# Spandan7724/Audio-Watermarking-Deep-Learning-Watermarks-for-Authenticating-Speech

Hardware: AMD Instinct MI355X
Metric: 1-s@16kHz clips/sec (gen+det+loss fwd-bwd) (higher is better)
Workload: dtype f32; 1 GPU; main16 train step: Generator+Detector+6 losses fwd-bwd + Adam, B=256 clips/GPU x 1 GPU, 1-s @ 16 kHz, message_bits=16 (BASELINE configs[2]); batch_per_gpu=256, global_batch=256, clip_len=16000, optimizer=fused flat Adam (wm_adam_step), parallelism=single

## Files before the change

audio-watermarking-deep-learning-watermarks-for-authenticating-speech_amd/csrc/small_convs.hip:

```cpp
#include "wm_common.hpp"
using namespace wm;

namespace {

__global__ __launch_bounds__(256) void stem_fwd_kernel(const float* __restrict__ s, const float* __restrict__ w,
                                                       const float* __restrict__ bias, float* __restrict__ y, int T) {
    __shared__ float ss[1024 + 8];
    __shared__ float ws[64 * 8];
    const int tilesPerClip = (T + 1023) / 1024;
    const int b = blockIdx.x / tilesPerClip, t0 = (blockIdx.x % tilesPerClip) * 1024;
    const float* sb = s + (size_t)b * T;
    for (int i = threadIdx.x; i < 1024 + 6; i += 256) {
        const int t = t0 - 3 + i;
        ss[i] = (t >= 0 && t < T) ? sb[t] : 0.f;
    }
    for (int i = threadIdx.x; i < 512; i += 256) {
        const int co = i >> 3, j = i & 7;
        ws[i] = (j < 7) ? w[co * 7 + j] : bias[co];
    }
    __syncthreads();
    const int t = t0 + 4 * threadIdx.x;
    if (t >= T) return;
    float v[10];
#pragma unroll
// ... 372 lines not shown
    for (int i = tid; i < OB * 64; i += 256) ws[i] = (i < NO * 64) ? w[i] : 0.f;
    for (int i = tid; i < 256 * GS; i += 256) gsm[i] = 0.f;
    const int tilesPerClip = (T + 255) / 256, ntiles = B * tilesPerClip;
    f32x16 accw[NT][2];
#pragma unroll
    for (int mt = 0; mt < NT; ++mt)
#pragma unroll
        for (int r = 0; r < 16; ++r) { accw[mt][0][r] = 0.f; accw[mt][1][r] = 0.f; }
    float accb = 0.f;
    constexpr int NG4 = (256 * NOMAX + 3) / 4, NGV = (NG4 + 255) / 256;
    float4 sx[16], sgv[NGV];
    auto load_piece = [&](int tile, int p) {
        const int b = tile / tilesPerClip, t0 = (tile % tilesPerClip) * 256;
        if (p < 16) {
            const int i = tid + p * 256, c = i >> 6, q = i & 63;
            sx[p] = *reinterpret_cast<const float4*>(x + ((size_t)b * 64 + c) * T + min(t0 + 4 * q, T - 4));
        } else {
            const float4* gb4 = reinterpret_cast<const float4*>(g + ((size_t)b * T + t0) * NO);
            const int lim4 = ((T - t0 < 256 ? T - t0 : 256) * NO) / 4;
            sgv[p - 16] = gb4[min(tid + (p - 16) * 256, lim4 - 1)];
        }
    };
    auto load_tile = [&](int tile) {
#pragma unroll
        for (int p = 0; p < 16 + NGV; ++p) load_piece(tile, p);
    };
    auto write_tile = [&](int tile) {
        const int t0 = (tile % tilesPerClip) * 256;
        const int nt = min(256, T - t0);
        const int row = tile / tilesPerClip;
        long long msg = 0;
        if constexpr (DL) msg = (row < BL) ? message[row] : 0;
        const float yl = row < BL ? 1.f : 0.f;
#pragma unroll
        for (int k = 0; k < 16; ++k) {
            const int i = tid + k * 256, c = i >> 6, q = i & 63;
            float4 v = sx[k];
            if (4 * q >= nt) v = make_float4(0.f, 0.f, 0.f, 0.f);
            float* d = xs + c * XS + 4 * q;
            d[0] = v.x; d[1] = v.y; d[2] = v.z; d[3] = v.w;
        }
#pragma unroll
        for (int k = 0; k < NGV; ++k) {
            const int f = tid + k * 256;
            if (f < NG4) {
                const float e[4] = {sgv[k].x, sgv[k].y, sgv[k].z, sgv[k].w};
#pragma unroll
                for (int j = 0; j < 4; ++j) {
                    const int i = 4 * f + j;
                    if (i < 256 * NO) {
                        const int r = NOC > 0 ? i / NO : div_small(i, magic), o = i - r * NO;
                        float val = e[j];
                        if constexpr (DL) {
                            if (o == 0) val = bce_logits_grad(val, yl, kl);
                            else val = (row < BL) ? bce_logits_grad(val, (float)((msg >> (o - 1)) & 1), kb) : 0.f;
                        }
                        gsm[r * GS + o] = (i < nt * NO) ? val : 0.f;
                    }
                }
            }
        }
    };
    int tile = blockIdx.x;
    if (tile < ntiles) load_tile(tile);
    __syncthreads();
    if (tile < ntiles) write_tile(tile);
    __syncthreads();
    while (tile < ntiles) {
        const int next = tile + gridDim.x, nextc = min(next, ntiles - 1);
        const int b = tile / tilesPerClip, t0 = (tile % tilesPerClip) * 256;
        const int nt = min(256, T - t0);
        {
            f32x16 acc[2][2];
#pragma unroll
            for (int mt = 0; mt < 2; ++mt)
#pragma unroll
                for (int n2 = 0; n2 < 2; ++n2)
#pragma unroll
                    for (int r = 0; r < 16; ++r) acc[mt][n2][r] = 0.f;
#pragma unroll
            for (int s = 0; s < (NOMAX + 1) / 2; ++s) {
                if (s < KS) {
                    const float a0 = ws[(2 * s + half) * 64 + l31], a1 = ws[(2 * s + half) * 64 + 32 + l31];
                    const float b0 = gsm[(wave * 64 + l31) * GS + 2 * s + half], b1 = gsm[(wave * 64 + 32 + l31) * GS + 2 * s + half];
                    acc[0][0] = mfma32(a0, b0, acc[0][0]); acc[0][1] = mfma32(a0, b1, acc[0][1]);
                    acc[1][0] = mfma32(a1, b0, acc[1][0]); acc[1][1] = mfma32(a1, b1, acc[1][1]);
                }
            }
            float* dxb = dx + (size_t)b * 64 * T + t0;
#pragma unroll
            for (int mt = 0; mt < 2; ++mt)
#pragma unroll
                for (int n2 = 0; n2 < 2; ++n2)
#pragma unroll
                    for (int r = 0; r < 16; ++r) {
                        const int c = mt * 32 + mfma_row(r, half), tt = wave * 64 + n2 * 32 + l31;
                        if (tt < nt) dxb[(size_t)c * T + tt] = acc[mt][n2][r];
                    }
        }
        {
            const float* ap = gsm + (wave * 64 + half) * GS + l31;
            const float* bp = xs + l31 * XS + wave * 64 + half;
#pragma unroll
            for (int s = 0; s < 32; ++s) {
                if (s < 16 + NGV) load_piece(nextc, s);
#pragma unroll
                for (int mt = 0; mt < NT; ++mt) {
                    const float a = ap[2 * s * GS + mt * 32];
                    accw[mt][0] = mfma32(a, bp[2 * s], accw[mt][0]);
                    accw[mt][1] = mfma32(a, bp[32 * XS + 2 * s], accw[mt][1]);
                }
            }
        }
        if ((tid & (OB - 1)) < NO) {
            const float* gp = gsm + (tid / OB) * OB * GS + (tid & (OB - 1));
#pragma unroll 8
            for (int tt = 0; tt < OB; ++tt) accb += gp[tt * GS];
        }
        __syncthreads();
        if (next < ntiles) write_tile(next);
        __syncthreads();
        tile = next;
    }
    __syncthreads();
    float* red = xs;
    for (int wv = 0; wv < 4; ++wv) {
        if (wave == wv) {
#pragma unroll
            for (int mt = 0; mt < NT; ++mt)
#pragma unroll
                for (int n2 = 0; n2 < 2; ++n2)
#pragma unroll
                    for (int r = 0; r < 16; ++r) {
                        const int o = mt * 32 + mfma_row(r, half), c = n2 * 32 + l31;
                        red[o * 64 + c] = (wv == 0) ? accw[mt][n2][r] : red[o * 64 + c] + accw[mt][n2][r];
                    }
        }
        __syncthreads();
    }
    float* out = partial + (size_t)blockIdx.x * (NO * 64 + NO);
    for (int i = tid; i < NO * 64; i += 256) out[i] = red[i];
    __syncthreads();
    red[tid] = ((tid & (OB - 1)) < NO) ? accb : 0.f;
    __syncthreads();
    if (tid < NO) {
        if constexpr (NT == 1)
            out[NO * 64 + tid] = ((red[tid] + red[32 + tid]) + (red[64 + tid] + red[96 + tid])) +
                                 ((red[128 + tid] + red[160 + tid]) + (red[192 + tid] + red[224 + tid]));
        else
            out[NO * 64 + tid] = (red[tid] + red[64 + tid]) + (red[128 + tid] + red[192 + tid]);
    }
}

}

extern "C" {

int wm_stem_fwd(const float* s, const float* w, const float* bias, float* y, int B, int T, hipStream_t stream) {
    if (T & 3) return (int)hipErrorInvalidValue;
    hipLaunchKernelGGL(stem_fwd_kernel, dim3(B * ((T + 1023) / 1024)), dim3(256), 0, stream, s, w, bias, y, T);
    WM_CHECK_LAUNCH();
    return 0;
}

#ifndef WM_STEM_WGS_PER_CU
#define WM_STEM_WGS_PER_CU 2
#endif
int wm_stem_bwd(const float* g, const float* s, const float* w, float* ds, float* partial, float* dw, float* db, int B,
                int T, int nds, int accumulate, hipStream_t stream) {
    if (T & 3) return (int)hipErrorInvalidValue;
    constexpr size_t lds = (size_t)(64 * 264 + 296 + 4 * 256) * sizeof(float);
    static wm::DevOnce attr_done;
    if (int rc = wm::lds_opt_in(reinterpret_cast<const void*>(stem_bwd_kernel), lds, attr_done)) return rc;
    const int ntiles = B * ((T + 255) / 256);
    const int grid = ntiles < WM_STEM_WGS_PER_CU * kNumCU ? ntiles : WM_STEM_WGS_PER_CU * kNumCU;
    hipLaunchKernelGGL(stem_bwd_kernel, dim3(grid), dim3(256), lds, stream, g, s, w, ds, partial, B, T, nds);
    WM_CHECK_LAUNCH();
    hipLaunchKernelGGL(stem_reduce_kernel, dim3(8), dim3(1024), 0, stream, (const float*)partial, grid, dw, db, accumulate);
    WM_CHECK_LAUNCH();
    return 0;
}

int wm_head1_fwd(const float* x, const float* w, const float* bias, float* y, int B, int T, hipStream_t stream) {
    if (T & 3) return (int)hipErrorInvalidValue;
    const int total4 = B * (T / 4);
    hipLaunchKernelGGL(head1_fwd_kernel, dim3((total4 + 255) / 256), dim3(256), 0, stream, x, w, bias, y, T / 4, total4);
    WM_CHECK_LAUNCH();
    return 0;
}

int wm_head1_tail_fwd(const float* x, const float* y2, const float* scale, const float* shift, const float* w, const float* bias,
                      float* out, void* mask, float* y, int B, int T, hipStream_t stream) {
    if ((T & 3) || B <= 0 || !y2 || !out) return (int)hipErrorInvalidValue;
    const int T4 = T / 4, grid = B * ((T4 + 255) / 256);
    if (mask) hipLaunchKernelGGL(head1_tail_fwd_kernel<true>, dim3(grid), dim3(256), 0, stream, x, y2, scale, shift, out, (unsigned*)mask, w, bias, y, T4);
    else hipLaunchKernelGGL(head1_tail_fwd_kernel<false>, dim3(grid), dim3(256), 0, stream, x, y2, scale, shift, out, (unsigned*)nullptr, w, bias, y, T4);
    WM_CHECK_LAUNCH();
    return 0;
}

int wm_head1_bwd(const float* g, const float* x, const float* w, float* dx, float* partial, float* dw, float* db, int B,
                 int T, int accumulate, hipStream_t stream) {
    if (T & 3) return (int)hipErrorInvalidValue;
    const int total4 = B * (T / 4);
    int grid = (total4 + 255) / 256;
    if (grid > 1024) grid = 1024;
    if (dx) hipLaunchKernelGGL(head1_bwd_kernel<true>, dim3(grid), dim3(256), 0, stream, g, x, w, dx, partial, T / 4, total4);
    else hipLaunchKernelGGL(head1_bwd_kernel<false>, dim3(grid), dim3(256), 0, stream, g, x, w, dx, partial, T / 4, total4);
    WM_CHECK_LAUNCH();
    hipLaunchKernelGGL(reduce_partials_kernel, dim3(1), dim3(256), 0, stream, (const float*)partial, grid, 65, 64, dw, accumulate);
    WM_CHECK_LAUNCH();
    hipLaunchKernelGGL(reduce_partials_kernel, dim3(1), dim3(256), 0, stream, (const float*)partial + 64, grid, 65, 1, db, accumulate);
    WM_CHECK_LAUNCH();
    return 0;
}

}

namespace {
struct HeadNFwd {
    const float *x, *y2, *scale, *shift, *w, *bias;
    float *out, *y, *partial;
    unsigned* mask;
    const long long* message;
    int BL, R, T, NO;
};
template <int NOC, bool TAIL, bool LOSS>
int launch_headN_fwd(const HeadNFwd& a, hipStream_t stream) {
    const size_t lds = (size_t)256 * (NOC > 0 ? NOC : (a.NO | 1)) * sizeof(float);
    if constexpr (NOC == 0) {
        static wm::DevOnce done;
        if (int rc = wm::lds_opt_in(reinterpret_cast<const void*>(headN_fwd_kernel<NOC, TAIL, LOSS>), 256 * 65 * sizeof(float), done)) return rc;
    }
    const unsigned magic = (unsigned)((0x100000000ull + a.NO - 1) / a.NO);
    hipLaunchKernelGGL((headN_fwd_kernel<NOC, TAIL, LOSS>), dim3(a.R * ((a.T + 255) / 256)), dim3(256), lds, stream, a.x, a.y2, a.scale,
                       a.shift, a.out, a.mask, a.w, a.bias, a.y, a.message, a.BL, a.partial, a.T, a.NO, magic);
    WM_CHECK_LAUNCH();
    return 0;
}
template <bool TAIL, bool LOSS>
int launch_headN_fwd_width(const HeadNFwd& a, hipStream_t stream) {
    if (a.NO == 17) return launch_headN_fwd<17, TAIL, LOSS>(a, stream);
    if (a.NO == 1) return launch_headN_fwd<1, TAIL, LOSS>(a, stream);
    return launch_headN_fwd<0, TAIL, LOSS>(a, stream);
}
}

extern "C" {

int wm_headN_fwd(const float* x, const float* w, const float* bias, float* y, int B, int T, int NO, hipStream_t stream) {
    if (NO < 1 || NO > 64 || B <= 0 || T <= 0) return (int)hipErrorInvalidValue;
    const HeadNFwd a{x, nullptr, nullptr, nullptr, w, bias, nullptr, y, nullptr, nullptr, nullptr, 0, B, T, NO};
    return launch_headN_fwd_width<false, false>(a, stream);
}

int wm_headN_tail_fwd(const float* x, const float* y2, const float* scale, const float* shift, const float* w, const float* bias,
                      const long long* message, int B, float* partial, float* loc_out, float* bce_out, float* out, void* mask,
                      float* logits, int R, int T, int NO, hipStream_t stream) {
    if (NO < 1 || NO > 64 || R <= 0 || T <= 0) return (int)hipErrorInvalidValue;
    if (y2 && (!scale || !shift || !out)) return (int)hipErrorInvalidValue;
    if (message && (B < 0 || B > R || !partial || !loc_out || (NO > 1 && !bce_out))) return (int)hipErrorInvalidValue;
    const HeadNFwd a{x, y2, scale, shift, w, bias, out, logits, partial, y2 ? (unsigned*)mask : nullptr, message, B, R, T, NO};
    const int rc = y2 ? (message ? launch_headN_fwd_width<true, true>(a, stream) : launch_headN_fwd_width<true, false>(a, stream))
                      : (message ? launch_headN_fwd_width<false, true>(a, stream) : launch_headN_fwd_width<false, false>(a, stream));
    if (rc || !message) return rc;
    const int grid = R * ((T + 255) / 256);
    WM_TRY((hipError_t)wm::launch_sum_scale2(partial, grid, 1.0 / ((double)R * T), loc_out, stream));
    if (NO > 1) WM_TRY((hipError_t)wm::launch_sum_scale2(partial + grid, grid, 1.0 / ((double)B * T * (NO - 1)), bce_out, stream));
    return 0;
}

}

namespace {
struct HeadNBwd {
    const float *g, *x, *w;
    float *dx, *partial;
    const long long* message;
    const float *g_loc, *g_bce;
    int BL, R, T, NO;
};
template <int NOC, int NT, bool DL>
int launch_headN_bwd(const HeadNBwd& a, int grid, hipStream_t stream) {
    constexpr size_t lds = (size_t)(64 * 257 + 256 * (32 * NT + 1) + 32 * NT * 64) * sizeof(float);
    static wm::DevOnce done;
    if (int rc = wm::lds_opt_in(reinterpret_cast<const void*>(headN_bwd_kernel<NOC, NT, DL>), lds, done)) return rc;
    const unsigned magic = a.NO > 1 ? (unsigned)((0x100000000ull + a.NO - 1) / a.NO) : 0u;
    hipLaunchKernelGGL((headN_bwd_kernel<NOC, NT, DL>), dim3(grid), dim3(256), lds, stream, a.g, a.x, a.w, a.dx, a.partial, a.R, a.T, a.NO,
                       magic, a.message, a.g_loc, a.g_bce, a.BL);
    WM_CHECK_LAUNCH();
    return 0;
}
template <bool DL>
int headN_bwd(const HeadNBwd& a, float* dw, float* db, int accumulate, hipStream_t stream) {
    const int NO = a.NO;
    if (NO < 1 || NO > 64) return (int)hipErrorInvalidValue;
    const int ntiles = a.R * ((a.T + 255) / 256);
    const int grid = ntiles < kNumCU ? ntiles : kNumCU;
    int rc;
    if (NO == 17) rc = launch_headN_bwd<17, 1, DL>(a, grid, stream);
    else if (NO == 1) rc = launch_headN_bwd<1, 1, DL>(a, grid, stream);
    else if (NO <= 32) rc = launch_headN_bwd<0, 1, DL>(a, grid, stream);
    else rc = launch_headN_bwd<0, 2, DL>(a, grid, stream);
    if (rc) return rc;
    const int n = NO * 64 + NO;
    hipLaunchKernelGGL(reduce_partials_kernel, dim3((NO * 64 + 63) / 64), dim3(256), 0, stream, (const float*)a.partial, grid, n, NO * 64, dw, accumulate);
    WM_CHECK_LAUNCH();
    hipLaunchKernelGGL(reduce_partials_kernel, dim3(1), dim3(256), 0, stream, (const float*)a.partial + NO * 64, grid, n, NO, db, accumulate);
    WM_CHECK_LAUNCH();
    return 0;
}
}

extern "C" {

int wm_headN_bwd(const float* g, const float* x, const float* w, float* dx, float* partial, float* dw, float* db, int B,
                 int T, int NO, int accumulate, hipStream_t stream) {
    const HeadNBwd a{g, x, w, dx, partial, nullptr, nullptr, nullptr, 0, B, T, NO};
    return headN_bwd<false>(a, dw, db, accumulate, stream);
}

int wm_headN_bwd_bce(const float* logits, const long long* message, const float* g_loc, const float* g_bce, const float* x,
                     const float* w, float* dx, float* partial, float* dw, float* db, int B, int R, int T, int NO, int accumulate,
                     hipStream_t stream) {
    if (!message || !g_loc || !g_bce || B < 0 || B > R) return (int)hipErrorInvalidValue;
    const HeadNBwd a{logits, x, w, dx, partial, message, g_loc, g_bce, B, R, T, NO};
    return headN_bwd<true>(a, dw, db, accumulate, stream);
}

}
```

audio-watermarking-deep-learning-watermarks-for-authenticating-speech_amd/ops.py:

```python
from __future__ import annotations

import contextlib
import os

import torch

from ._host import _chk, _chk_int, _chk_positive, _f32, _p, _seed64, _stream
from ._lib import lib

NCU = 256
BN_EPS = 1e-5
BN_MOMENTUM = 0.1


def _frames(x: torch.Tensor, name: str, ch: int) -> torch.Tensor:
    x = _chk(x, name, 3)
    if x.shape[1] != ch:
        raise ValueError(f"{name}: expected {ch} channels, got shape {tuple(x.shape)}")
    if x.shape[2] % 4 != 0:
        raise ValueError(f"{name}: clip length must be a multiple of 4 samples, got {x.shape[2]}")
    return x


_GRAD = {"on": True}
# ... 124 lines not shown
def switches(**values):
    prev = {name: _LIVE[SWITCHES[name][0]][SWITCHES[name][1]] for name in values}
    try:
        for name, value in values.items():
            set_switch(name, value)
        yield
    finally:
        for name, value in prev.items():
            set_switch(name, value)


def set_conv_bf_schedule(schedule: int):
    set_switch("schedule", schedule)


def set_conv_bf16x6(on: bool):
    set_switch("bf16x6", on)


def set_fused_backward(on: bool):
    set_switch("fused_bwd", on)


def set_mask_on_load(on: bool):
    set_switch("mask_on_load", on)


def set_bwd_f16x3(on: bool):
    set_switch("bwd_f16x3", on)


def set_fwd_f16x3(on: bool):
    set_switch("fwd_f16x3", on)


def set_eval_f16x3(on: bool):
    set_switch("eval_f16x3", on)


def pack_w64_h(w: torch.Tensor, mode: int) -> torch.Tensor:
    wph = torch.empty(2 * 3 * 4096 + 4, dtype=torch.int16, device=w.device)
    lib.wm_pack_w64_h(_p(w), _p(wph), mode, _stream())
    return wph


def set_pair_fold(on: bool):
    set_switch("pair_fold", on)


def set_resblock_one_launch(on: bool):
    set_switch("one_launch_eval", on)


def conv_bf16x6() -> bool:
    return _CONV["bf16x6"]


def pack_w64_bf(w: torch.Tensor, mode: int) -> torch.Tensor:
    wpb = torch.empty(3 * 3 * 4096, dtype=torch.int16, device=w.device)
    lib.wm_pack_w64_bf(_p(w), _p(wpb), mode, _stream())
    return wpb


def set_conv7_f16x3(on: bool):
    set_switch("conv7_f16x3", on)


def pack_w64_h7(w: torch.Tensor, mode: int) -> torch.Tensor:
    wph = torch.empty(2 * 7 * 4096 + 4, dtype=torch.int16, device=w.device)
    lib.wm_pack_w64_h7(_p(w), _p(wph), mode, _stream())
    return wph


def set_lstm_fwd_wave_specialised(on: bool):
    set_switch("lstm_fwd_ws", on)


def set_lstm_bwd_wave_specialised(on: bool):
    set_switch("lstm_bwd_ws", on)


_HEADS = {"tail_in_head": os.environ.get("WM_TAIL_IN_HEAD", "1") == "1"}


def set_tail_in_head(on: bool):
    _HEADS["tail_in_head"] = bool(on)


def read_tail_in_consumer(environ) -> bool:
    return environ.get("WM_TAIL_IN_CONSUMER", "1") == "1"


_TAILC = {"on": read_tail_in_consumer(os.environ)}


def set_tail_in_consumer(on: bool):
    _TAILC["on"] = bool(on)


def read_lstm_dx_in_bwd(environ) -> bool:
    return environ.get("WM_LSTM_DX_IN_BWD", "1") == "1"


_LSTM_DX = {"in_bwd": read_lstm_dx_in_bwd(os.environ)}


def set_lstm_dx_in_bwd(on: bool):
    _LSTM_DX["in_bwd"] = bool(on)


def read_head1_rank1(environ) -> bool:
    return environ.get("WM_HEAD1_RANK1", "1") == "1"


_HEAD1_R1 = {"on": read_head1_rank1(os.environ)}


def set_head1_rank1(on: bool):
    _HEAD1_R1["on"] = bool(on)


def head1_rank1_applies(x) -> bool:
    return bool(_HEAD1_R1["on"] and x.is_cuda and x.dim() == 3 and x.shape[-1] % 64 == 0 and _CONV["bf16x6"] and _CONV["fused_bwd"]
                and _CONV["bwd_f16x3"] and _CONV["mask_on_load"] and not _ASYNC["on"])


def _tail_in_consumer_launches(x, lstm: bool = False) -> bool:
    ok = (_TAILC["on"] and x.is_cuda and x.dim() == 3 and x.shape[-1] % 128 == 0 and _CONV["bf16x6"] and _CONV["fwd_f16x3"]
          and _CONV["schedule"] == 2)
    return bool(ok and (not lstm or (_LSTM["fused"] and _LSTM["fwd_ws"])))


def tail_in_consumer_applies(x, lstm: bool = False) -> bool:
    return _tail_in_consumer_launches(x, lstm) and bool(pair_node_applies(x))


def read_stem_in_conv1(environ) -> bool:
    return environ.get("WM_STEM_IN_CONV1", "1") == "1"


_STEMC = {"on": read_stem_in_conv1(os.environ)}


def set_stem_in_conv1(on: bool):
    _STEMC["on"] = bool(on)


def _stem_in_conv1_launches(s) -> bool:
    return bool(_STEMC["on"] and s.dim() == 3 and s.shape[1] == 1 and s.dtype == torch.float32 and _tail_in_consumer_launches(s))


def stem_in_conv1_applies(s, lstm: bool = False) -> bool:
    return _stem_in_conv1_launches(s) and tail_in_consumer_applies(s, lstm)


def _stem_in_dwgrad_launches(x) -> bool:
    return bool(_STEMC["on"] and _CONV["bwd_f16x3"] and x.shape[-1] % 64 == 0)


def set_gconv_f16x3(on: bool):
    set_switch("gconv_f16x3", on)


_GMAX = {}


def _note_gmax(t: torch.Tensor, maxes: torch.Tensor, per_clip: bool = False):
    import weakref
    if len(_GMAX) > 256:
        _GMAX.clear()
    _GMAX[id(t)] = (weakref.ref(t), t._version, maxes, per_clip)


def _noted(t: torch.Tensor, pop: bool):
    e = _GMAX.pop(id(t), None) if pop else _GMAX.get(id(t))
    return e if e is not None and e[0]() is t and e[1] == t._version else None


def gscale_of(g: torch.Tensor, log2_target: float = 12.0) -> torch.Tensor:
    e = _noted(g, pop=True)
    if e is not None:
        gsc = _f32(2, device=g.device)
        lib.wm_gscale_from_max(_p(e[2]), e[2].numel(), float(log2_target), _p(gsc), _stream())
        return gsc
    return gscale_absmax(g, log2_target)


_ZPOOL = {"buf": None, "used": 0}


def zeroed_slots(n: int, device) -> torch.Tensor:
    p = _ZPOOL
    if p["buf"] is None or p["buf"].device != torch.device(device) or p["used"] + n > p["buf"].numel():
        p["buf"], p["used"] = torch.zeros(max(1 << 16, n), dtype=torch.float32, device=device), 0
    s = p["buf"][p["used"]:p["used"] + n]
    p["used"] += n
    return s


def amax_per_clip(x: torch.Tensor) -> torch.Tensor:
    e = _noted(x, pop=False)
    if e is not None and e[3]:
        return e[2]
    NB = x.shape[0]
    m = zeroed_slots(NB, x.device)
    lib.wm_absmax_rows(_p(x), NB, x.numel() // NB, _p(m), _stream())
    _note_gmax(x, m, per_clip=True)
    return m


def gscale_absmax(g: torch.Tensor, log2_target: float = 12.0) -> torch.Tensor:
    gsc, scratch = _f32(2, device=g.device), _f32(1024, device=g.device)
    lib.wm_gscale_absmax(_p(g), g.numel(), _p(scratch), float(log2_target), _p(gsc), _stream())
    return gsc


def pack_w64_bf7(w: torch.Tensor, mode: int) -> torch.Tensor:
    wpb = torch.empty(3 * 7 * 4096, dtype=torch.int16, device=w.device)
    lib.wm_pack_w64_bf7(_p(w), _p(wpb), mode, _stream())
    return wpb


def _conv3(x, x2, w, mode, pa, pb, pc, bias, e1, ea, eb, y, stats, B, T, pro, epi):
    if _CONV["bf16x6"]:
        h = (_CONV["fwd_f16x3"] and mode == 0 and (pro, epi) in ((0, 0), (1, 0), (1, 4)) and _CONV["schedule"] == 2 and T % 128 == 0)
        lib.wm_conv64_bf(_p(x), _p(x2), _p(pack_w64_h(w, 0) if h else pack_w64_bf(w, mode)), _p(pa), _p(pb), _p(pc), _p(bias), _p(e1),
                         _p(ea), _p(eb), _p(y), _p(stats), B, T, pro, epi, 1 if h else 0, _stream())
    else:
        lib.wm_conv64(_p(x), _p(x2), _p(pack_w64(w, 3, mode)), _p(pa), _p(pb), _p(pc), _p(bias), _p(e1), _p(ea), _p(eb), _p(y),
                      _p(stats), B, T, 3, pro, epi, _stream())


def pack_w64(w: torch.Tensor, kw: int, mode: int) -> torch.Tensor:
    wp = _f32(kw * 4096, device=w.device)
    lib.wm_pack_w64(_p(w), _p(wp), kw, mode, _stream())
    return wp


def _resblock_fwd(x, params, training, want_grad, tail=True, pending=None, stem=None):
    w1, b1, g1, be1, w2, b2, g2, be2, rm1, rv1, nbt1, rm2, rv2, nbt2 = params
    if pending is not None:
        px, py2, pcst = pending[0], pending[2], pending[4]
        x, pmask = torch.empty_like(px), _tail_mask(px, want_grad)
    if stem is not None:
        ss, sw, sb = stem
        x = _f32(ss.shape[0], 64, ss.shape[2], device=ss.device)
        if not (training and _stem_in_conv1_launches(ss)):
            lib.wm_stem_fwd(_p(ss), _p(sw), _p(sb), _p(x), ss.shape[0], ss.shape[2], _stream())
            stem = None
    x = _frames(x, "ResBlock input", 64)
    B, _, T = x.shape
    dev, st = x.device, _stream()
    out = torch.empty_like(x) if tail else None
    cst = _f32(8, 64, device=dev)
    sc1, sh1, mu1, is1, sc2, sh2, mu2, is2 = cst.unbind(0)
    if training:
        y1, y2 = torch.empty_like(x), torch.empty_like(x)
        stats = _f32(NCU * 128, device=dev)
        if pending is not None:
            lib.wm_conv64_bf_tail(_p(px), _p(py2), _p(pack_w64_h(w1, 0)), _p(pcst[4]), _p(pcst[5]), _p(b1), _p(x), _p(pmask), _p(y1),
                                  _p(stats), B, T, st)
        elif stem is not None:
            lib.wm_conv64_bf_stem(_p(ss), _p(sw), _p(sb), _p(pack_w64_h(w1, 0)), _p(b1), _p(x), _p(y1), _p(stats), B, T, st)
        else:
            _conv3(x, None, w1, 0, None, None, None, b1, None, None, None, y1, stats, B, T, 0, 0)
        lib.wm_bn_finalize(_p(stats), NCU, float(B * T), _p(g1), _p(be1), _p(rm1), _p(rv1), _p(nbt1), BN_MOMENTUM, BN_EPS,
                           _p(sc1), _p(sh1), _p(mu1), _p(is1), st)
        _conv3(y1, None, w2, 0, sc1, sh1, None, b2, None, None, None, y2, stats, B, T, 1, 0)
        lib.wm_bn_finalize(_p(stats), NCU, float(B * T), _p(g2), _p(be2), _p(rm2), _p(rv2), _p(nbt2), BN_MOMENTUM, BN_EPS,
                           _p(sc2), _p(sh2), _p(mu2), _p(is2), st)
    else:
        lib.wm_bn_eval_scale_shift(_p(g1), _p(be1), _p(rm1), _p(rv1), BN_EPS, _p(sc1), _p(sh1), st)
        lib.wm_bn_eval_scale_shift(_p(g2), _p(be2), _p(rm2), _p(rv2), BN_EPS, _p(sc2), _p(sh2), st)
        if not want_grad and _CONV["bf16x6"] and _CONV["one_launch_eval"]:
            h = _CONV["eval_f16x3"]
            wp1 = torch.empty((2 * 3 * 4096 + 4) if h else 3 * 3 * 4096, dtype=torch.int16, device=dev)
            wp2 = torch.empty_like(wp1)
            pack = lib.wm_pack_w64_h_scaled if h else lib.wm_pack_w64_bf_scaled
            pack(_p(w1), _p(sc1), _p(wp1), st)
            pack(_p(w2), _p(sc2), _p(wp2), st)
            lib.wm_resblock_eval_bf(_p(x), _p(wp1), _p(wp2), _p(b1), _p(sc1), _p(sh1), _p(b2), _p(sc2), _p(sh2), _p(out), B, T,
                                    1 if h else 0, st)
            return out, None
        y1 = torch.empty_like(x)
        _conv3(x, None, w1, 0, None, None, None, b1, None, None, None, y1, None, B, T, 0, 0)
        if not want_grad and _CONV["bf16x6"] and _CONV["schedule"] == 2 and T % 128 == 0:
            _conv3(y1, None, w2, 0, sc1, sh1, None, b2, x, sc2, sh2, out, None, B, T, 1, 4)
            return out, None
        y2 = torch.empty_like(x)
        _conv3(y1, None, w2, 0, sc1, sh1, None, b2, None, None, None, y2, None, B, T, 1, 0)
        mu1.copy_(rm1); is1.copy_(torch.rsqrt(rv1 + BN_EPS)); mu2.copy_(rm2); is2.copy_(torch.rsqrt(rv2 + BN_EPS))
    more = () if pending is None else (pmask,)
    if not tail:
        return (None, (x, y1, y2, None, cst, w1, w2, g1, g2)) + more
    if want_grad:
        mask = torch.empty(B * 64 * ((T + 31) // 32), dtype=torch.int32, device=dev)
        lib.wm_bn_add_relu_mask(_p(x), _p(y2), _p(sc2), _p(sh2), _p(out), _p(mask), B, T, st)
    else:
        mask = None
        lib.wm_bn_add_relu(_p(x), _p(y2), _p(sc2), _p(sh2), _p(out), B, T, st)
    return (out, (x, y1, y2, mask, cst, w1, w2, g1, g2)) + more


class ResBlockFn(GradAwareFunction):

    @staticmethod
# ... 769 lines not shown
```

include/wm_hip.h:

```cpp
#ifndef WM_HIP_H
#define WM_HIP_H

#ifdef __cplusplus
extern "C" {
#endif

typedef struct ihipStream_t* wm_stream_t;


int wm_pack_w64(const float* w, float* wp, int KW, int mode, wm_stream_t stream);

int wm_conv64(const float* x, const float* x2, const float* wp, const float* pa, const float* pb, const float* pc,
              const float* bias, const float* e1, const float* ea, const float* eb, float* y, float* stats,
              int B, int T, int KW, int pro, int epi, wm_stream_t stream);

int wm_pack_w64_bf(const float* w, void* wpb, int mode, wm_stream_t stream);
int wm_set_conv_bf_schedule(int schedule, wm_stream_t stream);
int wm_conv64_bf(const float* x, const float* x2, const void* wpb, const float* pa, const float* pb, const float* pc,
                 const float* bias, const float* e1, const float* ea, const float* eb, float* y, float* stats,
                 int B, int T, int pro, int epi, int arith, wm_stream_t stream);
int wm_conv64_bf_tail(const float* x, const float* y2, const void* wpb_h, const float* sc2, const float* sh2, const float* bias,
                      float* out, void* mask, float* y, float* stats, int B, int T, wm_stream_t stream);

int wm_conv64_bf_stem(const float* s, const float* stem_w, const float* stem_b, const void* wpb_h, const float* bias, float* y0,
                      float* y, float* stats, int B, int T, wm_stream_t stream);

int wm_pack_w64_bf_scaled(const float* w, const float* row_scale, void* wpb, wm_stream_t stream);
int wm_resblock_eval_bf(const float* x, const void* w1pb, const void* w2pb, const float* b1, const float* sc1, const float* sh1,
                        const float* b2, const float* sc2, const float* sh2, float* y, int B, int T, int arith, wm_stream_t stream);
int wm_pack_w64_h_scaled(const float* w, const float* row_scale, void* wph, wm_stream_t stream);

int wm_dwgrad64_bf(const float* g, const float* g2, const float* ga, const float* gb, const float* gc, const void* wpb,
                   const float* x, const float* xa, const float* xb, const float* e1, const float* ea, const float* eb,
                   float* y, float* stats, float* partial, float* dw, float* dbias, int B, int T, int xpro, int epi, int accumulate,
                   const void* gmask, int arith, const float* gscale, float* dzmax, wm_stream_t stream);
int wm_pack_w64_h(const float* w, void* wph, int mode, wm_stream_t stream);
int wm_dwgrad64_bf_r1(const float* g, const float* g2, const float* ga, const float* gb, const float* gc, const void* wpb,
                      const float* x, const float* xa, const float* xb, const float* e1, const float* ea, const float* eb,
                      float* y, float* stats, float* partial, float* dw, float* dbias, int B, int T, int xpro, int epi, int accumulate,
                      const void* gmask, int arith, const float* gscale, float* dzmax, const float* g1, const float* hw,
                      wm_stream_t stream);
int wm_dwgrad64_bf_stem(const float* g, const float* g2, const float* ga, const float* gb, const float* gc, const void* wpb,
                        const float* e1, float* y, float* partial, float* dw, float* dbias, int B, int T, int accumulate,
                        const float* gscale, float* dzmax, const float* s, const float* stem_w, const float* stem_b,
                        wm_stream_t stream);

int wm_pack_w64_bf7(const float* w, void* wpb, int mode, wm_stream_t stream);
int wm_conv64_bf7(const float* x, const void* wpb, const float* vec, const float* bias, float* y, int B, int T, int pro, int epi,
                  int arith, const float* gscale, wm_stream_t stream);
int wm_pack_w64_h7(const float* w, void* wph, int mode, wm_stream_t stream);
int wm_gscale_absmax(const float* x, long long n, float* scratch, float log2_target, float* gscale, wm_stream_t stream);
int wm_gscale_from_max(const float* maxes, int n, float log2_target, float* gscale, wm_stream_t stream);
int wm_absmax_rows(const float* x, int rows, long long row_len, float* out, wm_stream_t stream);

int wm_wgrad64_bf7(const float* g, const float* x, const float* vec, float* partial, float* dw, float* dbias, int B, int T,
                   int xpro, int accumulate, int arith, const float* gscale, wm_stream_t stream);

int wm_wgrad64_bf(const float* g, const float* g2, const float* ga, const float* gb, const float* gc,
                  const float* x, const float* xa, const float* xb, float* partial, float* dw, float* dbias,
                  int B, int T, int gpro, int xpro, int accumulate, wm_stream_t stream);

int wm_wgrad64(const float* g, const float* g2, const float* ga, const float* gb, const float* gc,
               const float* x, const float* xa, const float* xb, float* partial, float* dw, float* dbias,
               int B, int T, int KW, int gpro, int xpro, int layout, int accumulate, wm_stream_t stream);

int wm_bn_finalize(const float* partials, int nparts, double count, const float* gamma, const float* beta,
                   float* running_mean, float* running_var, long long* num_batches_tracked, float momentum, float eps,
                   float* scale, float* shift, float* save_mean, float* save_invstd, wm_stream_t stream);
int wm_bn_eval_scale_shift(const float* gamma, const float* beta, const float* running_mean, const float* running_var,
                           float eps, float* scale, float* shift, wm_stream_t stream);
int wm_bn_add_relu(const float* x, const float* y2, const float* scale, const float* shift, float* out, int B, int T,
                   wm_stream_t stream);
int wm_relu_bwd_reduce(const float* g, const float* out, const float* y2, float* dz, float* partial, int B, int T,
                       wm_stream_t stream);
int wm_bn_add_relu_mask(const float* x, const float* y2, const float* scale, const float* shift, float* out, void* mask, int B, int T,
                        wm_stream_t stream);
int wm_relu_bwd_reduce_mask(const float* g, const void* mask, const float* y2, float* dz, float* partial, float* dzmax, int B, int T,
                            wm_stream_t stream);
int wm_relu_bwd_reduce_mask_r1(const float* g1, const float* w, const void* mask, const float* y2, float* partial, float* dzmax, int B,
                               int T, wm_stream_t stream);
int wm_bn_bwd_finalize(const float* partials, int nparts, double count, const float* gamma, const float* save_mean,
                       const float* save_invstd, float* A, float* Bc, float* Cc, float* dgamma, float* dbeta,
                       int accumulate, int eval_mode, const float* dzmax, int nmax, float* gscale, wm_stream_t stream);

int wm_stem_fwd(const float* s, const float* w, const float* bias, float* y, int B, int T, wm_stream_t stream);
int wm_stem_bwd(const float* g, const float* s, const float* w, float* ds, float* partial, float* dw, float* db, int B,
                int T, int nds, int accumulate, wm_stream_t stream);
int wm_head1_fwd(const float* x, const float* w, const float* bias, float* y, int B, int T, wm_stream_t stream);
int wm_head1_bwd(const float* g, const float* x, const float* w, float* dx, float* partial, float* dw, float* db, int B,
                 int T, int accumulate, wm_stream_t stream);
int wm_headN_fwd(const float* x, const float* w, const float* bias, float* y, int B, int T, int NO, wm_stream_t stream);
int wm_headN_bwd(const float* g, const float* x, const float* w, float* dx, float* partial, float* dw, float* db, int B,
                 int T, int NO, int accumulate, wm_stream_t stream);
int wm_head1_tail_fwd(const float* x, const float* y2, const float* scale, const float* shift, const float* w, const float* bias,
                      float* out, void* mask, float* y, int B, int T, wm_stream_t stream);
int wm_headN_tail_fwd(const float* x, const float* y2, const float* scale, const float* shift, const float* w, const float* bias,
                      const long long* message, int B, float* partial, float* loc_out, float* bce_out, float* out, void* mask,
                      float* logits, int R, int T, int NO, wm_stream_t stream);
int wm_headN_bwd_bce(const float* logits, const long long* message, const float* g_loc, const float* g_bce, const float* x,
                     const float* w, float* dx, float* partial, float* dw, float* db, int B, int R, int T, int NO, int accumulate,
                     wm_stream_t stream);

int wm_lstm_xproj(const float* x, const float* w_ih, const float* b_ih, const float* b_hh, float* xp, int B, int T,
                  wm_stream_t stream);
int wm_lstm_fwd(const float* xp, const float* w_hh, float* hout, float* gates, float* cst, int B, int T, wm_stream_t stream);
int wm_lstm_fwd_fused(const float* x, const float* w_ih, const float* b_ih, const float* b_hh, const float* w_hh,
                      float* hout, float* gates, float* cst, int B, int T, wm_stream_t stream);
int wm_set_lstm_fwd_wave_specialised(int on, wm_stream_t stream);
int wm_lstm_fwd_tail(const float* xres, const float* y2, const float* sc2, const float* sh2, float* out, void* mask, const float* w_ih,
                     const float* b_ih, const float* b_hh, const float* w_hh, float* hout, float* gates, float* cst, int B, int T,
                     wm_stream_t stream);
int wm_lstm_bwd(float* gates, const float* cst, const float* dh_out, const float* w_hh, int B, int T, wm_stream_t stream);
int wm_lstm_dx(const float* da, const float* w_ih, float* dx, int B, int T, wm_stream_t stream);
int wm_set_lstm_dx_bf16x6(int on, wm_stream_t stream);
int wm_lstm_bwd_fused(float* gates, const float* cst, const float* dh_out, const float* w_hh, const float* w_ih, float* dx,
                      int B, int T, wm_stream_t stream);
int wm_lstm_wgrad(const float* da, const float* x, const float* h, float* partial, float* dw_ih, float* dw_hh,
                  float* db_ih, float* db_hh, int B, int T, int accumulate, wm_stream_t stream);
int wm_lstm_bwd_wgrad(float* gates, const float* cst, const float* dh_out, const float* w_hh, const float* x, const float* h,
                      float* partial, float* dw_ih, float* dw_hh, float* db_ih, float* db_hh, int B, int T, int accumulate,
                      wm_stream_t stream);
int wm_lstm_bwd_wgrad_dx(const float* gates, const float* cst, const float* dh_out, const float* w_hh, const float* w_ih,
                         const float* x, const float* h, float* partial, float* dw_ih, float* dw_hh, float* db_ih, float* db_hh,
                         float* dx, int B, int T, int accumulate, wm_stream_t stream);

int wm_embed_gather(const float* table, const long long* message, float* vec, int B, int nrows, int* err, wm_stream_t stream);
int wm_embed_scatter_add(float* dtable, const long long* message, const float* dvec, int B, int nrows, wm_stream_t stream);
int wm_rowsum(const float* x, float* out, int rows, int T, wm_stream_t stream);

int wm_postproc_fwd(const float* d_in, const float* taps, int ntaps, float thr, float max_rms, float eps, int stages,
                    float* f_out, float* d_out, float* stats, int B, int T, wm_stream_t stream);
int wm_postproc_bwd(const float* g, const float* f_in, const float* stats, const float* taps, int ntaps, float thr,
                    float max_rms, int stages, float* d_raw, int B, int T, wm_stream_t stream);

int wm_mel_loss(const float* clean, const float* wm, const float* fb, const int* klo, const int* khi, const int* mlo,
                float* gframes, float* partial, float* loss_out, float* dsig, int B, int T, wm_stream_t stream);
int wm_loud_loss(const float* clean, const float* wm, float thresh, float* gframes, float* partial, float* loss_out,
                 float* dsig, int B, int T, wm_stream_t stream);
int wm_hf_penalty(const float* delta, int kcut, float* gframes, float* partial, float* loss_out, float* dsig, int B, int T,
                  wm_stream_t stream);

int wm_bce_fwd(const float* logits, const long long* message, float* partial, float* loc_out, float* bce_out, int B, int R,
               int T, int NO, wm_stream_t stream);
int wm_bce_bwd(const float* logits, const long long* message, const float* g_loc, const float* g_bce, float* dlogits, int B,
               int R, int T, int NO, wm_stream_t stream);
int wm_l1_fwd(const float* x, float* partial, float* out, long long n, wm_stream_t stream);
int wm_l1_bwd(const float* x, const float* g, float* dx, long long n, wm_stream_t stream);
int wm_adam_step(float* p, const float* g, float* m, float* v, long long n, double lr, double beta1, double beta2, double eps,
                 int step, wm_stream_t stream);

int wm_gconv(const float* x, const float* wp, const float* bias, const float* vec, const float* res, float* y, int NB,
             int Cin, int Lin, int K, int S, int P, int Mtot, int Nout, int st, int shp, int Cout, int Lout, int act,
             const float* x2, int Cin1, int nph, wm_stream_t stream);
int wm_gconv_h(const float* x, const void* wph, const float* bias, const float* vec, const float* res, float* y, int NB,
               int Cin, int Lin, int K, int S, int P, int Mtot, int Nout, int st, int shp, int Cout, int Lout, int act,
               const float* x2, int Cin1, int nph, const float* gscale, float* ymax, int per_clip, wm_stream_t stream);
int wm_gconv_pack_h(const float* wp, void* wph, float* scratch, int Cin, int K, int Mtot, wm_stream_t stream);
int wm_gconv_pack_h_conv(const float* w, void* wph, int Cout, int Cin, int K, int mode, wm_stream_t stream);
int wm_gwgrad_plan(int NB, int Ca, int Cb, int La, int K, long long* slab_floats, wm_stream_t stream);
int wm_gwgrad(const float* A, const float* Bx, float* G, float* dbias, float* slab, int NB, int Ca, int Cb, int La, int Lb,
              int K, int P, long long b_clip_stride, int remap, int r1, int r2, int accumulate, wm_stream_t stream);
int wm_gather_taps(const float* x, float* y, int NB, int C, int Lin, int K, int S, int P, int Lout, int order, wm_stream_t stream);
int wm_elu_bwd(const float* g, const float* y, float* dz, long long n, wm_stream_t stream);
int wm_channel_sum(const float* x, float* out, float* partial, int NB, int C, int L, int accumulate, wm_stream_t stream);
int wm_rowsum_any(const float* x, float* out, int rows, int L, wm_stream_t stream);
int wm_rows_scatter_add(float* dtable, const long long* idx, const float* dvec, int Bn, int dim, int nrows, wm_stream_t stream);
int wm_permute_acl(const float* x, float* y, int A, int C, int L, wm_stream_t stream);
int wm_lstm_seq_fwd(float* xp, const float* whh, float* hs, float* cs, int T, int H, int B, int save, wm_stream_t stream);
int wm_lstm_seq_bwd(float* gates, const float* cs, const float* dout, const float* whhT, float* dc, int T, int H, int B,
                    wm_stream_t stream);

int wm_resample_plan(int P, int Q, int width, int W, long long* tile_periods, wm_stream_t stream);
int wm_resample(const float* x, const float* taps, const int* first, float* y, int C, long long N, int P, int Q, int width, int W,
                long long L, long long total, wm_stream_t stream);

int wm_resample_add(const float* d, const float* taps, const int* first, const float* x, float* out, float* up, int C, long long N,
                    long long Nd, int P, int Q, int width, int W, wm_stream_t stream);

int wm_resample_rows(const float* x, const float* taps, const int* first, float* y, long long rows, long long N, long long L, int P, int Q,
                     int width, int W, wm_stream_t stream);

int wm_biquad_plan(int warm, int* chunk_len, wm_stream_t stream);
int wm_biquad(const float* x, void* out, void* mask_out, const void* mask_in, float b0, float b1, float b2, float a1, float a2,
              long long rows, long long n, int warm, int mode, int clamp, int reverse, wm_stream_t stream);

int wm_distort_plan(long long rows, long long n, long long* scratch_floats, wm_stream_t stream);
int wm_distort(const float* x, float* y, float* stat, float* scratch, long long rows, long long n, long long row0, long long seed,
               long long draw, float gain_lo, float gain_hi, float snr_lo, float snr_hi, float p_noise, wm_stream_t stream);
int wm_distort_bwd(const float* dy, const float* x, const float* stat, float* dx, float* scratch, long long rows, long long n,
                   long long row0, long long seed, long long draw, int through, wm_stream_t stream);

int wm_mdct_codec_plan(long long n, int M, int* frames_per_workgroup, long long* workgroups_per_row, wm_stream_t stream);
int wm_mdct_codec(const float* x, float* y, void* codes_out, const void* mask_in, const float* snr_db, long long rows, long long n, int M,
                  int band, int kcut, float floor_step, int quantise, wm_stream_t stream);

int wm_fir_rows(const float* x, const float* h, float* y, long long rows, long long n, int K, long long h_stride, int reverse,
                wm_stream_t stream);

int wm_rir_synth(const float* params, float* h, long long rows, int K, float sample_rate, long long row0, long long seed, long long draw,
                 wm_stream_t stream);

int wm_time_warp(const float* x, const float* params, const float* tab, float* y, long long rows, long long n, int zeros, int res,
                 int adjoint, wm_stream_t stream);

int wm_wsola(const float* x, const float* rate, const float* win, float* y, int* delta, long long rows, long long n_in, long long n_out,
             int L, int S, int mode, wm_stream_t stream);

int wm_lpc_codec(const float* x, float* y, const float* coeffs_in, float* coeffs_out, void* codes_out, const void* mask_in,
                 const float* snr_db, const float* lag, const float* expand, long long rows, long long n, int L, int p, float floor_step,
                 int quantise, int adjoint, wm_stream_t stream);

int wm_stoi_plan(long long rows, long long n, long long* scratch_bytes, wm_stream_t stream);
int wm_stoi(const float* x, const float* y, float* d, int* kept, void* scratch, long long rows, long long n, wm_stream_t stream);

int wm_masking_plan(long long rows, long long n, long long* frames, long long* chunk, long long* scratch_bytes, wm_stream_t stream);
int wm_masking_fwd(const float* x, const float* y, const float* tables, float* nmr_db, float* over_db, int* counts, float* coef,
                   void* scratch, long long rows, long long n, wm_stream_t stream);
int wm_masking_bwd(const float* x, const float* y, const float* coef, const float* gout, float* gy, long long rows, long long n,
                   wm_stream_t stream);

int wm_splice(const float* a, const float* b, float* y, int* lab, long long rows, long long n, long long row0, long long seed,
              long long draw, int max_spans, float p_span, long long len_lo, long long len_hi, float p_original, float p_silence,
              wm_stream_t stream);
int wm_splice_bwd(const float* dy, const int* lab, float* da, long long rows, long long n, wm_stream_t stream);
int wm_bce_masked_fwd(const float* logits, const long long* message, const int* lab, float* partial, long long* count_out,
                      float* loc_out, float* bce_out, int B, int R, int T, int NO, wm_stream_t stream);
int wm_bce_masked_bwd(const float* logits, const long long* message, const int* lab, const long long* count, const float* g_loc,
                      const float* g_bce, float* dlogits, int B, int R, int T, int NO, wm_stream_t stream);
int wm_loc_score(const float* logits, const int* lab, float thr_logit, int* counts, int* pred, int R, int T, int NO,
                 int lab_rows, wm_stream_t stream);

int wm_clip_scores_plan(long long R, int T, int NO, long long* scratch_bytes, wm_stream_t stream);
int wm_clip_scores(const float* logits, const long long* message, float thr_logit, float* prob, float* llr, int* votes, long long* words,
                   int* biterr, void* scratch, long long B, long long R, int T, int NO, wm_stream_t stream);

int wm_clip_features_plan(long long rows, long long n, int sample_rate, int* frames, int* energy_frames, int* lds_bytes,
                          wm_stream_t stream);
int wm_clip_features(const float* x, const float* sos, const float* fb, const int* klo, const int* khi, const float* dct, float* feat,
                     int* counts, float* frames_out, long long rows, long long n, int sample_rate, int warm, wm_stream_t stream);

#ifdef __cplusplus
}
#endif
#endif
```

Measured before the change: 5790 clips/s.

## Add software-pipelined headN backward kernel overlapping next-tile loads with MFMA

Adds a new headN backward kernel that double-buffers the upstream gradient tile in LDS and prefetches the next tile's x and g into registers while the current tile's dx and dW MFMAs run. Stores for the next tile are interleaved into the MFMA loops using sched barriers, so global-load latency is meant to hide behind compute instead of stalling between tiles. The kernel is on by default for NT==1 and NO!=1, with an env/runtime switch. It uses more LDS and many more registers for the prefetch buffers, which may reduce occupancy, and it applies only to the detector head backward, a small part of the step.

After: 5822 clips/s (median of 6 runs). No clear change (+0.6%).

```diff
diff --git a/audio-watermarking-deep-learning-watermarks-for-authenticating-speech_amd/csrc/small_convs.hip b/audio-watermarking-deep-learning-watermarks-for-authenticating-speech_amd/csrc/small_convs.hip
--- a/audio-watermarking-deep-learning-watermarks-for-authenticating-speech_amd/csrc/small_convs.hip
+++ b/audio-watermarking-deep-learning-watermarks-for-authenticating-speech_amd/csrc/small_convs.hip
@@ -548,7 +548,199 @@
     }
 }
 
-}
+template <int NOC, bool DL>
+__global__ __launch_bounds__(256) void headN_bwd_ovl_kernel(const float* __restrict__ g, const float* __restrict__ x,
+                                                            const float* __restrict__ w, float* __restrict__ dx,
+                                                            float* __restrict__ partial, int B, int T, int no, unsigned magic,
+                                                            const long long* __restrict__ message, const float* __restrict__ g_loc,
+                                                            const float* __restrict__ g_bce, int BL) {
+    constexpr int XS = 257, OB = 32, GS = OB + 1, GB = 256 * GS;
+    constexpr int NOMAX = NOC > 0 ? NOC : OB;
+    constexpr int KSC = (NOMAX + 1) / 2;
+    constexpr int XPS = (16 + KSC - 1) / KSC;
+    const int NO = NOC > 0 ? NOC : no;
+    const int KS = (NO + 1) / 2;
+    float kl = 0.f, kb = 0.f;
+    if constexpr (DL) {
+        kl = g_loc[0] / (float)((double)B * T);
+        kb = (NO > 1) ? g_bce[0] / (float)((double)BL * T * (NO - 1)) : 0.f;
+    }
+    extern __shared__ __align__(16) float smem[];
+    float* xs = smem;
+    float* gsm = xs + 64 * XS;
+    float* ws = gsm + 2 * GB;
+    const int tid = threadIdx.x, lane = tid & 63, wave = tid >> 6, half = lane >> 5, l31 = lane & 31;
+    for (int i = tid; i < OB * 64; i += 256) ws[i] = (i < NO * 64) ? w[i] : 0.f;
+    for (int i = tid; i < 2 * GB; i += 256) gsm[i] = 0.f;
+    const int tilesPerClip = (T + 255) / 256, ntiles = B * tilesPerClip;
+    f32x16 accw[2];
+#pragma unroll
+    for (int r = 0; r < 16; ++r) { accw[0][r] = 0.f; accw[1][r] = 0.f; }
+    float accb = 0.f;
+    constexpr int NG4 = (256 * NOMAX + 3) / 4, NGV = (NG4 + 255) / 256;
+    float4 sx[16], sgv[NGV];
+    auto load_x = [&](int tile, int k) {
+        const int b = tile / tilesPerClip, t0 = (tile % tilesPerClip) * 256;
+        const int i = tid + k * 256, c = i >> 6, q = i & 63;
+        sx[k] = *reinterpret_cast<const float4*>(x + ((size_t)b * 64 + c) * T + min(t0 + 4 * q, T - 4));
+    };
+    auto load_g = [&](int tile, int k) {
+        const int b = tile / tilesPerClip, t0 = (tile % tilesPerClip) * 256;
+        const float4* gb4 = reinterpret_cast<const float4*>(g + ((size_t)b * T + t0) * NO);
+        const int lim4 = ((T - t0 < 256 ? T - t0 : 256) * NO) / 4;
+        sgv[k] = gb4[min(tid + k * 256, lim4 - 1)];
+    };
+    auto write_x = [&](int nt, int k) {
+        const int i = tid + k * 256, c = i >> 6, q = i & 63;
+        float4 v = sx[k];
+        if (4 * q >= nt) v = make_float4(0.f, 0.f, 0.f, 0.f);
+        float* d = xs + c * XS + 4 * q;
+        d[0] = v.x; d[1] = v.y; d[2] = v.z; d[3] = v.w;
+    };
+    auto write_g = [&](int tile, int k, float* gd, int opq) {
+        const int nt = min(256, T - (tile % tilesPerClip) * 256);
+        const int row = tile / tilesPerClip;
+        long long msg = 0;
+        if constexpr (DL) msg = (row < BL) ? message[row] : 0;
+        const float yl = row < BL ? 1.f : 0.f;
+        const int f = tid + k * 256 + opq;
+        if (f < NG4) {
+            const float e[4] = {sgv[k].x, sgv[k].y, sgv[k].z, sgv[k].w};
+#pragma unroll
+            for (int j = 0; j < 4; ++j) {
+                const int i = 4 * f + j;
+                if (i < 256 * NO) {
+                    const int r = NOC > 0 ? i / NO : div_small(i, magic), o = i - r * NO;
+                    float val = e[j];
+                    if constexpr (DL) {
+                        const float y = (o == 0) ? yl : (float)((msg >> ((o - 1) & 63)) & 1);
+                        val = bce_logits_grad(val, y, (o == 0) ? kl : kb);
+                        if (o != 0 && row >= BL) val = 0.f;
+                    }
+                    gd[r * GS + o] = (i < nt * NO) ? val : 0.f;
+                }
+            }
+        }
+    };
+    int tile = blockIdx.x;
+    const int last = ntiles - 1;
+#pragma unroll
+    for (int k = 0; k < 16; ++k) load_x(min(tile, last), k);
+#pragma unroll
+    for (int k = 0; k < NGV; ++k) load_g(min(tile, last), k);
+    __syncthreads();
+#pragma unroll
+    for (int k = 0; k < NGV; ++k) {
+        write_g(min(tile, last), k, gsm, 0);
+        load_g(min(tile + (int)gridDim.x, last), k);
+    }
+    __syncthreads();
+    int p = 0;
+    while (tile < ntiles) {
+        const int nextc = min(tile + (int)gridDim.x, last), next2c = min(tile + 2 * (int)gridDim.x, last);
+        const int b = tile / tilesPerClip, t0 = (tile % tilesPerClip) * 256;
+        const int nt = min(256, T - t0);
+        const float* gc = gsm + p * GB;
+        float* gn = gsm + (p ^ 1) * GB;
+        int opq = 0;
+        if constexpr (NOC == 0) asm volatile("" : "+s"(opq));
+        {
+            f32x16 acc[2][2];
+#pragma unroll
+            for (int mt = 0; mt < 2; ++mt)
+#pragma unroll
+                for (int n2 = 0; n2 < 2; ++n2)
+#pragma unroll
+                    for (int r = 0; r < 16; ++r) acc[mt][n2][r] = 0.f;
+            const float* wp = ws + half * 64 + l31;
+            const float* gp0 = gc + (wave * 64 + l31) * GS + half;
+            float a0 = wp[0], a1 = wp[32], b0 = gp0[0], b1 = gp0[32 * GS];
+#pragma unroll
+            for (int s = 0; s < KSC; ++s) {
+                float na0 = 0.f, na1 = 0.f, nb0 = 0.f, nb1 = 0.f;
+                if (s + 1 < KSC) {
+                    na0 = wp[(s + 1) * 128]; na1 = wp[(s + 1) * 128 + 32];
+                    nb0 = gp0[2 * (s + 1)]; nb1 = gp0[32 * GS + 2 * (s + 1)];
+                }
+                __builtin_amdgcn_sched_barrier(0);
+                if (s < KS) {
+                    acc[0][0] = mfma32(a0, b0, acc[0][0]); acc[0][1] = mfma32(a0, b1, acc[0][1]);
+                    acc[1][0] = mfma32(a1, b0, acc[1][0]); acc[1][1] = mfma32(a1, b1, acc[1][1]);
+                }
+                __builtin_amdgcn_sched_barrier(0);
+#pragma unroll
+                for (int j = 0; j < XPS; ++j) {
+                    const int k = s * XPS + j;
+                    if (k < 16) { write_x(nt, k); load_x(nextc, k); }
+                }
+                a0 = na0; a1 = na1; b0 = nb0; b1 = nb1;
+            }
+            float* dxb = dx + (size_t)b * 64 * T + t0;
+#pragma unroll
+            for (int mt = 0; mt < 2; ++mt)
+#pragma unroll
+                for (int n2 = 0; n2 < 2; ++n2)
+#pragma unroll
+                    for (int r = 0; r < 16; ++r) {
+                        const int c = mt * 32 + mfma_row(r, half), tt = wave * 64 + n2 * 32 + l31;
+                        if (tt < nt) dxb[(size_t)c * T + tt] = acc[mt][n2][r];
+                    }
+        }
+        __syncthreads();
+        {
+            const float* ap = gc + (wave * 64 + half) * GS + l31;
+            const float* bp = xs + l31 * XS + wave * 64 + half;
+            const float* gp = gc + (tid / OB) * OB * GS + (tid & (OB - 1));
+            float a = ap[0], x0 = bp[0], x1 = bp[32 * XS], gv = gp[0];
+#pragma unroll
+            for (int s = 0; s < 32; ++s) {
+                float na = 0.f, nx0 = 0.f, nx1 = 0.f, ngv = 0.f;
+                if (s < 31) { na = ap[2 * (s + 1) * GS]; nx0 = bp[2 * (s + 1)]; nx1 = bp[32 * XS + 2 * (s + 1)]; ngv = gp[(s + 1) * GS]; }
+                __builtin_amdgcn_sched_barrier(0);
+                accw[0] = mfma32(a, x0, accw[0]);
+                accw[1] = mfma32(a, x1, accw[1]);
+                accb += gv;
+                __builtin_amdgcn_sched_barrier(0);
+                if (s >= 4 && (s - 4) % 3 == 0 && (s - 4) / 3 < NGV) {
+                    const int k = (s - 4) / 3;
+                    write_g(nextc, k, gn, opq);
+                    load_g(next2c, k);
+                }
+                a = na; x0 = nx0; x1 = nx1; gv = ngv;
+            }
+        }
+        __syncthreads();
+        tile += gridDim.x;
+        p ^= 1;
+    }
+    __syncthreads();
+    float* red = xs;
+    for (int wv = 0; wv < 4; ++wv) {
+        if (wave == wv) {
+#pragma unroll
+            for (int n2 = 0; n2 < 2; ++n2)
+#pragma unroll
+                for (int r = 0; r < 16; ++r) {
+                    const int o = mfma_row(r, half), c = n2 * 32 + l31;
+                    red[o * 64 + c] = (wv == 0) ? accw[n2][r] : red[o * 64 + c] + accw[n2][r];
+                }
+        }
+        __syncthreads();
+    }
+    float* out = partial + (size_t)blockIdx.x * (NO * 64 + NO);
+    for (int i = tid; i < NO * 64; i += 256) out[i] = red[i];
+    __syncthreads();
+    red[tid] = ((tid & (OB - 1)) < NO) ? accb : 0.f;
+    __syncthreads();
+    if (tid < NO)
+        out[NO * 64 + tid] = ((red[tid] + red[32 + tid]) + (red[64 + tid] + red[96 + tid])) +
+                             ((red[128 + tid] + red[160 + tid]) + (red[192 + tid] + red[224 + tid]));
+}
+
+}
+
+static int g_bwd_stage_overlap = 1;
+extern "C" int wm_set_bwd_stage_overlap(int on, hipStream_t) { g_bwd_stage_overlap = on ? 1 : 0; return 0; }
 
 extern "C" {
 
@@ -679,9 +871,20 @@
 template <int NOC, int NT, bool DL>
 int launch_headN_bwd(const HeadNBwd& a, int grid, hipStream_t stream) {
     constexpr size_t lds = (size_t)(64 * 257 + 256 * (32 * NT + 1) + 32 * NT * 64) * sizeof(float);
+    const unsigned magic = a.NO > 1 ? (unsigned)((0x100000000ull + a.NO - 1) / a.NO) : 0u;
+    if constexpr (NT == 1 && NOC != 1) {
+        if (g_bwd_stage_overlap) {
+            constexpr size_t lds2 = lds + (size_t)256 * 33 * sizeof(float);
+            static wm::DevOnce done2;
+            if (int rc = wm::lds_opt_in(reinterpret_cast<const void*>(headN_bwd_ovl_kernel<NOC, DL>), lds2, done2)) return rc;
+            hipLaunchKernelGGL((headN_bwd_ovl_kernel<NOC, DL>), dim3(grid), dim3(256), lds2, stream, a.g, a.x, a.w, a.dx, a.partial, a.R,
+                               a.T, a.NO, magic, a.message, a.g_loc, a.g_bce, a.BL);
+            WM_CHECK_LAUNCH();
+            return 0;
+        }
+    }
     static wm::DevOnce done;
     if (int rc = wm::lds_opt_in(reinterpret_cast<const void*>(headN_bwd_kernel<NOC, NT, DL>), lds, done)) return rc;
-    const unsigned magic = a.NO > 1 ? (unsigned)((0x100000000ull + a.NO - 1) / a.NO) : 0u;
     hipLaunchKernelGGL((headN_bwd_kernel<NOC, NT, DL>), dim3(grid), dim3(256), lds, stream, a.g, a.x, a.w, a.dx, a.partial, a.R, a.T, a.NO,
                        magic, a.message, a.g_loc, a.g_bce, a.BL);
     WM_CHECK_LAUNCH();
diff --git a/audio-watermarking-deep-learning-watermarks-for-authenticating-speech_amd/ops.py b/audio-watermarking-deep-learning-watermarks-for-authenticating-speech_amd/ops.py
--- a/audio-watermarking-deep-learning-watermarks-for-authenticating-speech_amd/ops.py
+++ b/audio-watermarking-deep-learning-watermarks-for-authenticating-speech_amd/ops.py
@@ -300,6 +300,22 @@
 
 def stem_in_conv1_applies(s, lstm: bool = False) -> bool:
     return _stem_in_conv1_launches(s) and tail_in_consumer_applies(s, lstm)
+
+
+def read_bwd_stage_overlap(environ) -> bool:
+    return environ.get("WM_BWD_STAGE_OVERLAP", "1") == "1"
+
+
+_BWD_OVL = {"on": read_bwd_stage_overlap(os.environ)}
+
+
+def set_bwd_stage_overlap(on: bool):
+    lib.wm_set_bwd_stage_overlap(int(bool(on)), None)
+    _BWD_OVL["on"] = bool(on)
+
+
+if "WM_BWD_STAGE_OVERLAP" in os.environ:
+    set_bwd_stage_overlap(_BWD_OVL["on"])
 
 
 def _stem_in_dwgrad_launches(x) -> bool:
diff --git a/include/wm_hip.h b/include/wm_hip.h
--- a/include/wm_hip.h
+++ b/include/wm_hip.h
@@ -100,6 +100,7 @@
 int wm_headN_bwd_bce(const float* logits, const long long* message, const float* g_loc, const float* g_bce, const float* x,
                      const float* w, float* dx, float* partial, float* dw, float* db, int B, int R, int T, int NO, int accumulate,
                      wm_stream_t stream);
+int wm_set_bwd_stage_overlap(int on, wm_stream_t stream);
 
 int wm_lstm_xproj(const float* x, const float* w_ih, const float* b_ih, const float* b_hh, float* xp, int B, int T,
                   wm_stream_t stream);
```
